# UnaryPlus/raytrace

Measured on AMD Instinct MI355X. Metric: Msamples/s (pixels×spp/s) + achieved HBM GB/s, Cornell-box 600×600, higher is better.
Workload: dtype f64; 1 GPU; cornell 600x600 200spp depth 50; width=600, height=600, spp=200, max_depth=50, parallelism=rows interleaved over 1 GPU(s), row_block 1

## Files before the change

### raytrace_amd/csrc/rt_build.cpp

```cpp
#include <algorithm>
#include <cmath>
#include <cstdarg>
#include <cstdio>
#include <cstdlib>
#include <cstring>
#include <optional>
#include <utility>

#include "../../include/rt.h"
#include "rt_bvh.h"
#include "rt_encode8_table.h"
#include "rt_internal.h"
#include "rt_kernel_class.h"

const char* rt_knob(const char* name) {
  const char* on = std::getenv("RT_AMD_EXPERIMENTS");
  if (!on || !*on || std::atoi(on) == 0) return nullptr;
  return std::getenv(name);
}

namespace {

struct d3 {
  double x, y, z;
// ... 1020 lines not shown
  P.tile_rows = rows;
  return RT_OK;
}

template <class R>
int rt_host_match_target(const HostScene& H, int variant, KernelParamsT<R>& P) {
  P.target_defer = 0;
  P.target_rec = -1;
  if (!H.flat || (variant & RT_VAR_BASE) != RT_VAR_FLAT || (variant & (RT_VAR_MATS | RT_VAR_MEDIA))) return 0;
  if (const char* e = rt_knob("RT_AMD_TARGET_DEFER"))
    if (atoi(e) == 0) return 0;
  if (rt_knob("RT_AMD_VARIANT")) return 0;
  const HostArraysT<R>& A = H.arrays<R>();
  if (P.n_targets != 1 || H.n_media != 0 || A.flat_recs.empty() || A.prim_shade.empty()) return 0;
  const DevFlatSet& S = H.flat_sets[0];
  const DevTargetT<R>& T = P.targets[0];
  for (int k = S.first; k < S.end_quad; ++k) {
    const R* f = A.flat_recs.data() + 16 * (size_t)k;
    if (std::memcmp(f, T.n, 3 * sizeof(R)) || std::memcmp(f + 4, T.q, 3 * sizeof(R)) ||
        std::memcmp(f + 8, T.wa, 3 * sizeof(R)) || std::memcmp(f + 12, T.wb, 3 * sizeof(R)))
      continue;
    int kf, slot;
    std::memcpy(&kf, f + 3, 4);
    std::memcpy(&slot, f + 11, 4);
    if (kf != 1 || slot < 0 || slot >= (int)A.prim_shade.size()) continue;
    if (A.prim_shade[slot].kind >= 2) continue;
    P.target_defer = 1;
    P.target_rec = k;
    return 1;
  }
  return 0;
}

template <class R>
SceneRecordsT<R> rt_host_records(const HostScene& H) {
  const HostArraysT<R>& A = H.arrays<R>();
  SceneRecordsT<R> r;
  r.nodes = H.nodes.data(), r.perlin_perm = H.perlin_perm.data();
  r.prims = A.prims.data(), r.prim_uv = A.prim_uv.data(), r.motions = A.motions.data();
  r.uvframes = A.uvframes.data(), r.texels = A.texels.data(), r.perlin_grad = A.perlin_grad.data();
  r.flat_recs = A.flat_recs.data(), r.prim_shade = A.prim_shade.data(), r.mats = A.mats.data();
  r.texs = A.texs.data(), r.boxes = A.boxes.data(), r.instances = A.instances.data();
  return r;
}

template <class R>
int rt_host_render_params(const HostScene& H, int variant, const SceneRecordsT<R>& r, const rt_camera_settings* cs,
                          uint64_t seed, const rt_exec* ex, const LaunchInputs& L, KernelParamsT<R>& P,
                          std::string& err) {
  constexpr bool f64 = sizeof(R) == 8;
  const bool flat = (variant & RT_VAR_BASE) == RT_VAR_FLAT;
  std::memset(&P, 0, sizeof P);
  if (int rc = rt_host_make_params(cs, seed, ex, P, err)) return rc;
  P.nodes = r.nodes, P.perlin_perm = r.perlin_perm;
  P.prims = r.prims, P.prim_uv = r.prim_uv, P.motions = r.motions, P.uvframes = r.uvframes, P.texels = r.texels;
  P.perlin_grad = r.perlin_grad, P.flat_recs = r.flat_recs, P.prim_shade = r.prim_shade, P.mats = r.mats;
  P.texs = r.texs, P.boxes = r.boxes, P.instances = r.instances;
  P.surface_root = H.surface_root;
  P.leaf_exit_pct = f64 ? H.leaf_exit_pct64 : H.leaf_exit_pct;
  P.surface_prefix = !flat && H.n_nodes > 0 ? 1 : 0;
  P.n_media = H.n_media;
  for (int k = 0; k < H.n_media; ++k) P.media[k] = H.arrays<R>().media[k];
  for (int k = 0; k <= RT_MAX_MEDIA; ++k) P.flat_sets[k] = H.flat_sets[k];
  P.stack_depth = rt_host_stack_depth(H);
  P.lds_nodes = L.lds_nodes;
  P.n_prims = H.n_prims;
  P.pool_shift = L.pool_shift ? L.pool_shift : L.lone && flat ? 6 : 0;
  rt_host_plan_work(P, L.resident_lanes, flat, L.lone);
  if (L.flat_ring) rt_host_plan_ring(P, variant, L.lone, L.pool_shift, L.resident_lanes);
  P.trav_exit_pct = f64 ? H.trav_exit_pct64 : H.trav_exit_pct;
  P.out_frame_rows = L.out_frame_rows;
  P.sample0 = L.sample0;
  rt_host_match_target(H, variant, P);
  return RT_OK;
}
#define RT_INSTANTIATE(R)                                                                                           \
  template int rt_host_match_target<R>(const HostScene&, int, KernelParamsT<R>&);                                   \
  template SceneRecordsT<R> rt_host_records<R>(const HostScene&);                                                   \
  template int rt_host_render_params<R>(const HostScene&, int, const SceneRecordsT<R>&, const rt_camera_settings*, \
                                        uint64_t, const rt_exec*, const LaunchInputs&, KernelParamsT<R>&, std::string&);
RT_INSTANTIATE(float)
RT_INSTANTIATE(double)
#undef RT_INSTANTIATE

bool rt_host_media_late(const HostScene& H) {
  if (H.n_media == 0) return false;
  for (int m = 0; m < H.n_media; ++m) {
    const DevMediumT<double>& M = H.f64.media[m];
    if (!M.alias_surface && !(M.root < 0 && M.root != RT_EMPTY_ROOT)) return false;
  }
  return true;
}

FastDiv rt_host_fastdiv(uint32_t d) {
  FastDiv f{0u, 0, d, 0};
  if (d <= 1) return f;
  int l = 0;
  while ((1ull << l) < d) ++l;
  f.m = (uint32_t)((((1ull << 32) * ((1ull << l) - d)) / d) + 1);
  f.s = l - 1;
  return f;
}

template <class R>
void rt_host_plan_work(KernelParamsT<R>& P, long long resident_lanes, bool two_sizes, bool lone) {
  P.div_width = rt_host_fastdiv((uint32_t)P.cam.width);
  P.div_block = rt_host_fastdiv((uint32_t)P.row_block);
  const bool pool_given = P.pool_shift >= 4;
  if (!pool_given) P.pool_shift = __builtin_ctz(RT_POOL);
// ... 109 lines not shown
```

### raytrace_amd/csrc/rt_internal.h

```cpp
#pragma once
#include <stdint.h>

#include <string>
#include <vector>

#ifndef RT_BLOCK
#define RT_BLOCK 64
#endif
#ifndef RT_BLOCK_BVH
#define RT_BLOCK_BVH 256
#endif
#define RT_MAX_NODES (1 << 26)
#define RT_STACK_DEPTH 64
#define RT_MAX_MEDIA 8
#define RT_MAX_TARGETS 8
#ifndef RT_LEAF_MAX
#define RT_LEAF_MAX 8
#endif
#ifndef RT_POOL
#define RT_POOL 128
#endif
#ifndef RT_AGG_SLOTS_FLAT
#define RT_AGG_SLOTS_FLAT 8
#endif
#ifndef RT_AGG_PIX_FLAT
#define RT_AGG_PIX_FLAT 17
#endif
#ifndef RT_AGG_SLOTS_FLAT_F64
#define RT_AGG_SLOTS_FLAT_F64 7
#endif
#ifndef RT_AGG_PIX_FLAT_F64
#define RT_AGG_PIX_FLAT_F64 22
#endif
#ifndef RT_AGG_SLOTS_BVH
#define RT_AGG_SLOTS_BVH 4
#endif
#ifndef RT_AGG_PIX_BVH
#define RT_AGG_PIX_BVH 5
#endif
#define RT_RING_LANES 64
#define RT_RING_AGG_PIX 8
#define RT_RING_AGG_SLOTS_F64 6
#define RT_RING_AGG_SLOTS_F32 5
#ifndef RT_BIG_CHUNK_MAX
#define RT_BIG_CHUNK_MAX 16
#endif
#ifndef RT_BIG_CHUNK_MAX_ASYNC
#define RT_BIG_CHUNK_MAX_ASYNC 64
#endif
#ifndef RT_TAIL_ITEMS_F64
#define RT_TAIL_ITEMS_F64 16
#endif
#ifndef RT_TAIL_ITEMS_F32
#define RT_TAIL_ITEMS_F32 32
#endif
#ifndef RT_TAIL_ITEMS_ASYNC
#define RT_TAIL_ITEMS_ASYNC 8
#endif
#define RT_LEAF_SHIFT 6
#define RT_FLAT_MAX 32
#define RT_LDS_PRIMS_MAX 256
#define RT_PREFIX_MAX 16
#ifndef RT_PREFIX_AREA
#define RT_PREFIX_AREA 0.1
#endif
#ifndef RT_PREFIX_SHRINK
#define RT_PREFIX_SHRINK 0.25
#endif
#define RT_EMPTY_ROOT ((int)0x80000000)
#ifndef RT_GRID_RESERVE
#define RT_GRID_RESERVE 0
#endif
#define RT_INST_FLAG 0x40000000
#define RT_INST_EXIT 0x7FFFFFFF

#define RT_VAR_FLAT 0
// ... 136 lines not shown
  int chunk;
  int n_chunks;
  int n_items;
  int big_chunk;
  int n_big_chunks;
  int big_items;
  int small_start;
  FastDiv div_big, div_small;
  int agg_big, agg_small;
  int pool_shift;
  int stack_depth;
  int lds_nodes;
  int trav_exit_pct;
  int leaf_exit_pct;
  int n_prims;
  int surface_root;
  int surface_prefix;
  int n_media;
  int n_targets;
  R rem_prob;
  DevMediumT<R> media[RT_MAX_MEDIA];
  DevFlatSet flat_sets[1 + RT_MAX_MEDIA];
  DevTargetT<R> targets[RT_MAX_TARGETS];
  DevCameraT<R> cam;
  uint32_t key0, key1;
  int n_shards, shard, row_block, tile_rows;
  int out_frame_rows;
  FastDiv div_width, div_block;
  int sample0;
  int target_defer;
  int target_rec;
  int cam_defocus;
  int flat_ring;
};
using DevMaterial = DevMaterialT<float>;
using DevTexture = DevTextureT<float>;
using DevMedium = DevMediumT<float>;
using DevBox = DevBoxT<float>;
using DevTarget = DevTargetT<float>;
using DevCamera = DevCameraT<float>;
using DevInstance = DevInstanceT<float>;
using KernelParams = KernelParamsT<float>;
using KernelParams64 = KernelParamsT<double>;

#define RT_FIX_SCALE 4294967296.0
#define RT_ACC_WORDS(R) (sizeof(R) == 8 ? 6 : 3)

template <class R>
struct HostArraysT {
  std::vector<R> prims, prim_uv, motions, uvframes, texels, perlin_grad;
  std::vector<R> flat_recs;
  std::vector<DevMaterialT<R>> prim_shade, mats;
  std::vector<DevTextureT<R>> texs;
  std::vector<DevBoxT<R>> boxes;
  std::vector<DevInstanceT<R>> instances;
  DevMediumT<R> media[RT_MAX_MEDIA];
};
struct HostScene {
  std::vector<float> nodes;
  std::vector<int> perlin_perm;
  std::vector<int> prim_mat;
  HostArraysT<float> f32;
  HostArraysT<double> f64;
  int surface_root = RT_EMPTY_ROOT;
  int n_media = 0;
  DevFlatSet flat_sets[1 + RT_MAX_MEDIA] = {};
// ... 30 lines not shown
                    int stack_depth);
inline int rt_host_stack_depth(const HostScene& H) { return H.max_depth > 1 ? H.max_depth : 1; }
template <class R>
int rt_host_make_params(const rt_camera_settings* cs, uint64_t seed, const rt_exec* ex, KernelParamsT<R>& P,
                        std::string& err);
template <class R>
struct SceneRecordsT {
  const float* nodes = nullptr;
  const int* perlin_perm = nullptr;
  const R *prims = nullptr, *prim_uv = nullptr, *motions = nullptr, *uvframes = nullptr, *texels = nullptr;
  const R *perlin_grad = nullptr, *flat_recs = nullptr;
  const DevMaterialT<R>*prim_shade = nullptr, *mats = nullptr;
  const DevTextureT<R>* texs = nullptr;
  const DevBoxT<R>* boxes = nullptr;
  const DevInstanceT<R>* instances = nullptr;
};
template <class R>
SceneRecordsT<R> rt_host_records(const HostScene& H);
struct LaunchInputs {
  long long resident_lanes = 0;
  int lds_nodes = 0;
  bool lone = false;
  int sample0 = 0, out_frame_rows = 0;
  int pool_shift = 0;
  bool flat_ring = false;
};
template <class R>
int rt_host_render_params(const HostScene& H, int variant, const SceneRecordsT<R>& records,
                          const rt_camera_settings* cs, uint64_t seed, const rt_exec* ex, const LaunchInputs& L,
                          KernelParamsT<R>& P, std::string& err);
template <class R>
int rt_host_match_target(const HostScene& H, int variant, KernelParamsT<R>& P);
template <class R>
void rt_host_plan_work(KernelParamsT<R>& P, long long resident_lanes, bool two_sizes, bool lone = false);
template <class R>
bool rt_host_plan_ring(KernelParamsT<R>& P, int variant, bool lone, int pool_shift = 0, long long resident_lanes = 0);
FastDiv rt_host_fastdiv(uint32_t d);
void rt_host_encode8_thresholds(int encoding, double* thr);

int rt_render_resident_blocks(const KernelParams*, int device, int stack_depth, int variant, int lds_nodes);
int rt_render_resident_blocks(const KernelParams64*, int device, int stack_depth, int variant, int lds_nodes);
int rt_launch_render(const KernelParams& p, int grid_blocks, int variant, void* stream);
int rt_launch_render(const KernelParams64& p, int grid_blocks, int variant, void* stream);
int rt_launch_resolve(const KernelParams& p, void* stream);
int rt_launch_resolve(const KernelParams64& p, void* stream);
int rt_launch_features(const KernelParams& p, int variant, unsigned long long* feat, int n_feat, void* stream);
int rt_launch_features(const KernelParams64& p, int variant, unsigned long long* feat, int n_feat, void* stream);
struct rt_ray;
struct rt_hit;
int rt_launch_query(const KernelParams& p, int variant, const rt_ray* rays, rt_hit* hits, const int* prim_mat, long long n,
                    int flags, void* stream);
int rt_launch_query(const KernelParams64& p, int variant, const rt_ray* rays, rt_hit* hits, const int* prim_mat,
                    long long n, int flags, void* stream);
struct rt_adaptive_rec;
int rt_launch_list(const KernelParams& p, int variant, const rt_adaptive_rec* list, const int* n_list, int n_samples,
                   int chunk, void* stream);
int rt_launch_list(const KernelParams64& p, int variant, const rt_adaptive_rec* list, const int* n_list, int n_samples,
                   int chunk, void* stream);
#if defined(RT_PHASE_PROF)
int rt_prof_read_kernel(const KernelParams*, unsigned long long* out, int n);
int rt_prof_read_kernel(const KernelParams64*, unsigned long long* out, int n);
#endif
#if defined(RT_WAVE_STAMPS)
int rt_stamps_read_kernel(const KernelParams*, unsigned long long* out, int n_waves);
int rt_stamps_read_kernel(const KernelParams64*, unsigned long long* out, int n_waves);
#endif
// ... 3 lines not shown
```

### raytrace_amd/csrc/rt_kernel_class.h

```cpp
#pragma once
#include <stddef.h>
#include <type_traits>
#include "rt_internal.h"

struct KernelClass {
  int var, tex, media; bool mats, inst; int leaf; bool narrow;
};

#ifndef RT_WAVES_FLAT
#define RT_WAVES_FLAT 7
#endif
#ifndef RT_WAVES_FLAT_NOISE
#define RT_WAVES_FLAT_NOISE 5
#endif
#ifndef RT_WAVES_BVH
#define RT_WAVES_BVH 5
#endif
#ifndef RT_WAVES_FLAT_TEX0
#define RT_WAVES_FLAT_TEX0 8
#endif
#ifndef RT_WAVES_BVH_LITE
#define RT_WAVES_BVH_LITE 6
#endif
#ifndef RT_WAVES64_FLAT_LITE
// ... 65 lines not shown
#endif
constexpr bool rt_class_acc_lds(bool f64, KernelClass c) {
  return RT_ACC_IN_LDS && c.var != RT_VAR_FLAT && (f64 || !c.media);
}

constexpr bool rt_class_agg_wide(bool f64, KernelClass c) { return f64 || c.media == 0; }
constexpr int rt_class_agg_slots(bool f64, KernelClass c) {
  return c.var != RT_VAR_FLAT ? RT_AGG_SLOTS_BVH : rt_class_agg_wide(f64, c) ? RT_AGG_SLOTS_FLAT_F64 : RT_AGG_SLOTS_FLAT;
}
constexpr int rt_class_agg_pix(bool f64, KernelClass c) {
  return c.var != RT_VAR_FLAT ? RT_AGG_PIX_BVH : rt_class_agg_wide(f64, c) ? RT_AGG_PIX_FLAT_F64 : RT_AGG_PIX_FLAT;
}
static_assert(RT_AGG_SLOTS_FLAT < 255 && RT_AGG_SLOTS_FLAT_F64 < 255 && RT_AGG_SLOTS_BVH < 255,
              "slot + 1 must fit the 8 bits of rt_trace.h ItemCtx::tp");
constexpr int rt_acc_words(bool f64) { return f64 ? RT_ACC_WORDS(double) : RT_ACC_WORDS(float); }
constexpr int rt_class_agg_bytes(bool f64, KernelClass c) {
  return rt_class_agg_slots(f64, c) * (rt_class_agg_pix(f64, c) * rt_acc_words(f64) * 8 + 2 * 4);
}
constexpr size_t rt_class_fixed_lds(bool f64, KernelClass c) {
  const size_t block = (size_t)rt_class_block(f64, c);
  return (rt_class_acc_lds(f64, c) ? rt_acc_words(f64) * 8 * block : 0) + rt_class_agg_bytes(f64, c) * (block / 64);
}
constexpr size_t rt_class_lds_bytes(bool f64, KernelClass c, int stack_depth, int lds_nodes) {
  return rt_class_fixed_lds(f64, c) +
         (c.var == RT_VAR_FLAT ? 0 : (size_t)(stack_depth + 1) * rt_class_block(f64, c) * sizeof(int) + (size_t)lds_nodes * 64);
}

constexpr KernelClass rt_ring_class() { return KernelClass{RT_VAR_FLAT, 0, 0, false, false, 0, false}; }
constexpr bool rt_class_has_ring(KernelClass c) {
  return c.var == RT_VAR_FLAT && c.tex == 0 && c.media == 0 && !c.mats && !c.inst;
}
constexpr int rt_ring_agg_slots(bool f64) { return f64 ? RT_RING_AGG_SLOTS_F64 : RT_RING_AGG_SLOTS_F32; }
constexpr int rt_ring_agg_bytes(bool f64) { return rt_ring_agg_slots(f64) * (RT_RING_AGG_PIX * rt_acc_words(f64) * 8 + 2 * 4); }
constexpr int rt_ring_ray_bytes(bool f64) { return RT_RING_LANES * (6 * (f64 ? 8 : 4) + 4 * 4); }
constexpr size_t rt_ring_lds_bytes(bool f64) { return (size_t)rt_ring_ray_bytes(f64) + rt_ring_agg_bytes(f64); }
static_assert(RT_BLOCK == RT_RING_LANES, "the ring belongs to a one-wave workgroup");
static_assert(rt_ring_lds_bytes(false) <= rt_class_fixed_lds(false, rt_ring_class()) &&
                  rt_ring_lds_bytes(true) <= rt_class_fixed_lds(true, rt_ring_class()),
              "the ring form's LDS must not exceed the legacy kernel's (same workgroups per CU)");

#ifndef RT_NOLICM_FLAT_LITE
#define RT_NOLICM_FLAT_LITE 0
#endif
#ifndef RT_NOLICM_BVH_LITE
#define RT_NOLICM_BVH_LITE 0
#endif
constexpr bool rt_class_nolicm(bool f64, KernelClass c) {
  const bool heavy = c.tex != 0 || c.media != 0 || c.mats;
  return c.var == RT_VAR_FLAT ? f64 && (RT_NOLICM_FLAT_LITE || heavy) : RT_NOLICM_BVH_LITE || heavy || c.inst;
}

#ifndef RT_LEAF_MEDIA
#define RT_LEAF_MEDIA 1
#endif
constexpr bool rt_media_late_compiled(int var) { return var == RT_VAR_BVH; }
constexpr bool rt_leaf_compiled(int var, int tex, int media, bool inst, int leaf) {
  if (leaf == 0) return true;
  if (var != RT_VAR_BVH || inst) return false;
  return media ? RT_LEAF_MEDIA && tex == 0 && leaf == 1 : true;
}
constexpr bool rt_class_compiled(bool f64, KernelClass c) {
  if (c.var == RT_VAR_BVH_LOCKSTEP && !RT_LOCKSTEP_KERNELS) return false;
  if (c.var != RT_VAR_BVH && c.inst) return false;
  if (c.media == 2 && !rt_media_late_compiled(c.var)) return false;
  return rt_leaf_compiled(c.var, c.tex, c.media, c.inst, c.leaf) && (!c.narrow || rt_class_has_twin(f64, c));
}

// ... 40 lines not shown
```

### raytrace_amd/csrc/rt_render_kernel.h

```cpp
#include <hip/hip_runtime.h>
#include <stdint.h>

#include <type_traits>

#include "rt_kernel_class.h"
#include "rt_trace.h"

namespace RT_NS {

#if defined(RT_WAVE_STAMPS)
#define RT_STAMP_WAVES 16384
static __device__ unsigned long long rt_stamp_buf[4 * RT_STAMP_WAVES];
#endif

namespace {

static_assert(RT_POOL >= 64, "a refill must cover every lane of a wave");
#ifndef RT_QUEUES
#define RT_QUEUES 4
#endif
#ifndef RT_QUEUE_INTERLEAVE
#define RT_QUEUE_INTERLEAVE 1
#endif
static_assert((RT_QUEUES & (RT_QUEUES - 1)) == 0 && RT_QUEUES <= 8, "RT_QUEUES: a power of two, at most 8 (workspace)");
// ... 272 lines not shown
    rt_stamp_buf[4 * wave + 1] = work.t_drain;                                                    \
    rt_stamp_buf[4 * wave + 2] = wall_clock64();                                                  \
    rt_stamp_buf[4 * wave + 3] = (unsigned long long)__builtin_amdgcn_s_getreg((4 << 0) | (31 << 11)) << 32 | \
                                 (unsigned)__builtin_amdgcn_s_getreg((20 << 0) | (3 << 11));      \
  }
#else
#define RT_STAMP_END(work)
#endif
  if constexpr (kVar == RT_VAR_FLAT) {
    WaveWork<kSlots, kPix, true> work(P, wave, waves, agg);
    overflow = lane_loop_lockstep<true, kTex, kMedia != 0, kMats>(P, work, Trav{nullptr, 0, nullptr}, P.prims, acc);
    work.finish();
    RT_STAMP_END(work)
  } else {
    v4f* lds_nodes = reinterpret_cast<v4f*>(smem_rest + (P.stack_depth + 1) * block_nodes);
    const float4* src = reinterpret_cast<const float4*>(P.nodes);
    for (int i = threadIdx.x; i < 4 * P.lds_nodes; i += block_copy) {
      const float4 q = src[i];
      lds_nodes[i] = v4f{q.x, q.y, q.z, q.w};
    }
    __syncthreads();
    WaveWork<kSlots, kPix, RT_KARGS_WORK_BVH> work(P, wave, waves, agg);
    const Trav W{smem_rest + threadIdx.x, block_stack, lds_nodes};
    if constexpr (kVar == RT_VAR_BVH_LOCKSTEP)
      overflow = lane_loop_lockstep<false, kTex, kMedia != 0, kMats>(P, work, W, P.prims, acc);
    else
      overflow = lane_loop_bvh<kTex, kMedia, kMats, kInst, kLeaf>(P, work, W, P.prims, acc);
    work.finish();
    RT_STAMP_END(work)
  }
  if (overflow) atomicOr(P.status, 1);
}

#if !RT_TU_NOLICM
__global__ __launch_bounds__(RT_BLOCK) __attribute__((amdgpu_waves_per_eu(rt_class_waves(RT_F64, rt_ring_class()))))
void rt_render_kernel_ring(KernelParams P) {
  extern __shared__ int smem[];
  real* ring_od = reinterpret_cast<real*>(smem);
  uint32_t* ring_meta = reinterpret_cast<uint32_t*>(ring_od + 6 * RT_RING_LANES);
  unsigned long long* agg = reinterpret_cast<unsigned long long*>(ring_meta + 4 * RT_RING_LANES);
  constexpr int kAggBytes = rt_ring_agg_bytes(RT_F64);
  for (int i = (int)__lane_id(); i < kAggBytes / 8; i += 64) agg[i] = 0ull;
  WaveWork<rt_ring_agg_slots(RT_F64), RT_RING_AGG_PIX, true> work(P, (int)blockIdx.x, (int)gridDim.x, agg);
  lane_loop_flat_ring(P, work, ring_od, ring_meta);
  work.finish();
}
#endif

#ifndef RT_KERNEL_ONLY
#if !RT_TU_NOLICM
__global__ __launch_bounds__(256) void rt_resolve_kernel(const long long* __restrict__ accum,
                                                         const unsigned int* __restrict__ nanflag,
                                                         real* __restrict__ out, int n_pixels, int spp, double scale,
                                                         int width, int frame_rows, int n_shards, int shard,
                                                         int row_block) {
  const int i = blockIdx.x * 256 + threadIdx.x;
  if (i >= n_pixels) return;
  size_t w = 3 * (size_t)i + blockIdx.y;
  if (frame_rows > 0) {
    const int t = i / width, px = i - t * width;
    const int g = ((t / row_block) * n_shards + shard) * row_block + t % row_block;
    if (g >= frame_rows) return;
    w = 3 * ((size_t)g * width + px) + blockIdx.y;
  }
  const bool bad = nanflag[i] != 0u;
#if RT_F64
  (void)scale;
  const long long* a = accum + 6 * (size_t)i + blockIdx.y;
  const double sum = ((double)a[0] + (double)(unsigned long long)a[3] * (1.0 / RT_FIX_SCALE)) * (1.0 / RT_FIX_SCALE);
  out[w] = bad ? __builtin_nan("") : sum / (double)spp;
#else
  (void)spp;
  out[w] = bad ? __builtin_nanf("") : (float)((double)accum[3 * (size_t)i + blockIdx.y] * scale);
// ... 10 lines not shown
    return nullptr;
  });
}
render_fn render_kernel_nolicm(int variant);
template <class T, size_t N>
static int diag_read(T (&buf)[N], unsigned long long* out, size_t n) {
  if (hipMemcpyFromSymbol(out, HIP_SYMBOL(buf), n * sizeof(T)) != hipSuccess) return -1;
  void* p = nullptr;
  if (hipGetSymbolAddress(&p, HIP_SYMBOL(buf)) != hipSuccess) return -1;
  return hipMemset(p, 0, sizeof(buf)) == hipSuccess ? 0 : -1;
}
int diag_read_nolicm(int which, unsigned long long* out, size_t n);
static int diag_read_this_tu(int which, unsigned long long* out, size_t n) {
  (void)which, (void)out, (void)n;
#if defined(RT_PHASE_PROF)
  if (which == 0) return diag_read(rt_prof_buf, out, n);
#endif
#if defined(RT_WAVE_STAMPS)
  if (which == 1) return diag_read(rt_stamp_buf, out, n);
#endif
  return -1;
}
#if RT_TU_NOLICM
int diag_read_nolicm(int which, unsigned long long* out, size_t n) { return diag_read_this_tu(which, out, n); }
#endif
static int diag_read_both(int which, unsigned long long* out, size_t n) {
  if (hipDeviceSynchronize() != hipSuccess || diag_read_this_tu(which, out, n)) return -1;
  unsigned long long* other = new unsigned long long[n];
  const int rc = diag_read_nolicm(which, other, n);
  for (size_t k = 0; k < n && rc == 0; ++k) out[k] += other[k];
  delete[] other;
  return rc;
}
#if RT_TU_NOLICM
render_fn render_kernel_nolicm(int variant) { return render_kernel_this_tu(variant); }
#else
static render_fn render_kernel_of(int variant) {
  const render_fn f = render_kernel_this_tu(variant);
  return f ? f : render_kernel_nolicm(variant);
}
#endif

#endif
}
#if !defined(RT_KERNEL_ONLY) && !RT_TU_NOLICM

int rt_render_resident_blocks(const KernelParamsT<RT_NS::real>*, int device, int stack_depth, int variant,
                              int lds_nodes) {
  using namespace RT_NS;
  int per_cu = 0, cus = 0;
  const KernelClass c = rt_class_of(RT_F64, variant);
  size_t lds = rt_class_lds_bytes(RT_F64, c, stack_depth, lds_nodes);
  if (lds > 65536 && hipFuncSetAttribute((const void*)render_kernel_of(variant),
                                         hipFuncAttributeMaxDynamicSharedMemorySize, (int)lds) != hipSuccess)
    return -1;
  hipError_t e =
      hipOccupancyMaxActiveBlocksPerMultiprocessor(&per_cu, render_kernel_of(variant), rt_class_block(RT_F64, c), lds);
  if (e != hipSuccess) return -1;
  if (hipDeviceGetAttribute(&cus, hipDeviceAttributeMultiprocessorCount, device) != hipSuccess) return -1;
  if (per_cu < 1) per_cu = 1;
  return per_cu * cus;
}

int rt_launch_render(const KernelParamsT<RT_NS::real>& p, int grid_blocks, int variant, void* stream) {
  using namespace RT_NS;
  if (p.n_items <= 0 || grid_blocks <= 0) return 0;
  const KernelClass c = rt_class_of(RT_F64, variant);
  const int block = rt_class_block(RT_F64, c);
  long long need = ((long long)p.n_items + block - 1) / block;
  int grid = need < grid_blocks ? (int)need : grid_blocks;
  if (p.flat_ring) {
    if (!rt_class_has_ring(c)) return -1;
    hipLaunchKernelGGL(rt_render_kernel_ring, dim3(grid), dim3(block), rt_ring_lds_bytes(RT_F64), (hipStream_t)stream, p);
    return hipGetLastError() == hipSuccess ? 0 : -1;
  }
  size_t lds = rt_class_lds_bytes(RT_F64, c, p.stack_depth, p.lds_nodes);
  hipLaunchKernelGGL(render_kernel_of(variant), dim3(grid), dim3(block), lds, (hipStream_t)stream, p);
  return hipGetLastError() == hipSuccess ? 0 : -1;
}

#if defined(RT_PHASE_PROF)
int rt_prof_read_kernel(const KernelParamsT<RT_NS::real>*, unsigned long long* out, int n) {
  using namespace RT_NS;
  if (n > PF_N) n = PF_N;
  return diag_read_both(0, out, (size_t)n) == 0 ? n : -1;
}
#endif

#if defined(RT_WAVE_STAMPS)
int rt_stamps_read_kernel(const KernelParamsT<RT_NS::real>*, unsigned long long* out, int n_waves) {
  using namespace RT_NS;
  if (n_waves > RT_STAMP_WAVES) n_waves = RT_STAMP_WAVES;
  return diag_read_both(1, out, 4 * (size_t)n_waves) == 0 ? n_waves : -1;
}
#endif

int rt_launch_resolve(const KernelParamsT<RT_NS::real>& p, void* stream) {
  using namespace RT_NS;
  int n = p.tile_rows * p.cam.width;
  if (n <= 0) return 0;
  hipLaunchKernelGGL(rt_resolve_kernel, dim3((n + 255) / 256, 3), dim3(256), 0, (hipStream_t)stream,
                     (const long long*)p.accum, p.nanflag, p.out, n, p.cam.spp, 1.0 / (RT_FIX_SCALE * (double)p.cam.spp),
                     p.cam.width, p.out_frame_rows, p.n_shards, p.shard, p.row_block);
  return hipGetLastError() == hipSuccess ? 0 : -1;
}
#endif
// ... 1 lines not shown
```

### raytrace_amd/csrc/rt_trace.h

```cpp
#ifndef RT_TRACE_COMMON_H
#define RT_TRACE_COMMON_H
#include <stdint.h>

#include "../../include/rt.h"
#include "rt_internal.h"
#include "rt_sincos_table.h"

#ifdef RT_HOST_EMU
#include <cmath>
#include <cstring>
#define RT_FN static inline
#define RT_FN_SPEC inline
namespace rt_emu {
inline int f2i(float f) {
  int i;
  std::memcpy(&i, &f, 4);
  return i;
}
extern thread_local long long counters[4];
}
#define RT_F2I(f) rt_emu::f2i(f)
#define RT_COUNT(i) (++rt_emu::counters[i])
#define RT_ANY(x) (x)
#define RT_BALLOT_COUNT(x) ((x) ? 1 : 0)
// ... 1101 lines not shown
template <bool kDefer>
RT_FN void closest_flat(const KernelParams& P, int set, const RayCtx& R, real tmin, Closest& C, real* apdf = nullptr) {
  {
    const DevFlatSet& S = P.flat_sets[set];
    const real tmin_up = float_up(tmin);
    for (int b = S.box_first; b < S.box_end; ++b) test_box<true>((const RT_CAS DevBox*)P.boxes + b, R, tmin_up, C);
    int k = S.first;
    const RT_CAS PrimRec64* rp = (const RT_CAS PrimRec64*)P.flat_recs + k;
    for (; k < S.end_quad; ++k, ++rp) {
      if constexpr (kDefer) {
        if (k == P.target_rec) {
          real term;
          test_static<RT_PRIM_CLASS_QUAD>(ld_rec64(rp), R, tmin, tmin_up, C, 0, &term);
          *apdf = RFMA(P.targets[0].prob_icr, term, *apdf);
          continue;
        }
      }
      test_static<RT_PRIM_CLASS_QUAD>(ld_rec64(rp), R, tmin, tmin_up, C);
    }
    for (; k < S.end_tri; ++k, ++rp) test_static<RT_PRIM_CLASS_TRI>(ld_rec64(rp), R, tmin, tmin_up, C);
    for (; k < S.end_sphere; ++k, ++rp) test_static<RT_PRIM_CLASS_SPHERE>(ld_rec64(rp), R, tmin, tmin_up, C);
    for (; k < S.end; ++k, ++rp) test_rec<true>(P, ld_rec64(rp), k, R, tmin, tmin_up, C);
#if RT_F64
    if (C.t < kInf) C.prim = C.ord;
#else
    const uint32_t hi = (uint32_t)(C.key >> 32);
    if (hi < 0x7f800000u) {
      C.t = __builtin_bit_cast(real, hi);
      C.prim = (int)(uint32_t)C.key;
    }
#endif
  }
}
template <>
RT_FN_SPEC void closest<true>(const KernelParams& P, cfp prims, int root, int set, const RayCtx& R, real tmin, Closest& C,
                         const Trav& W, int* overflow) {
  (void)prims;
  (void)root;
  (void)W;
  (void)overflow;
  closest_flat<false>(P, set, R, tmin, C);
}

template <>
RT_FN_SPEC void closest<false>(const KernelParams& P, cfp prims, int root, int set, const RayCtx& R, real tmin,
                          Closest& C, const Trav& W, int* overflow) {
  TravState S;
  trav_begin(S, root, tmin);
  if (set == 0) prefix_hits(P, prims, R, tmin, S.C);
  while (!trav_done(S)) trav_round(P, R, S, W, *overflow RT_PROF_NULLARG);
  C = S.C;
}

#ifndef RT_KARGS_OPAQUE
#define RT_KARGS_OPAQUE 1
#endif
#if defined(RT_HOST_EMU) || !RT_KARGS_OPAQUE
#define RT_KARGS(P0) (P0)
#else
RT_FN const KernelParams& rt_kargs() {
  const RT_CAS KernelParams* pp = (const RT_CAS KernelParams*)__builtin_amdgcn_kernarg_segment_ptr();
  asm volatile("" : "+s"(pp));
  return *(const KernelParams*)pp;
}
#define RT_KARGS(P0) rt_kargs()
#endif
// ... 85 lines not shown
    medium_event(P, m, pix, sample, seg, lo, hi, tbest, hit_medium);
  }
}

RT_FN f3 normalize_fused(f3 v) {
#ifdef RT_HOST_EMU
  return normalize(v);
#else
  const real l = RFMA(v.z, v.z, RFMA(v.y, v.y, v.x * v.x));
#if RT_F64
  if (RABS(l) <= RL(1e-12) || RABS(RL(1.0) - l) <= RL(1e-12)) return v;
#else
  if (l <= RL(1e-12)) return v;
#endif
  return RT_RSQRT(l) * v;
#endif
}
template <bool kFlatLoop = false>
RT_FN f3 normal_plus_unit_vector(f3 n, uint32_t a, uint32_t b, f3& uu) {
  real z = RL(1.0) - RL(2.0) * u01(a);
  real r = RT_SQRT(RMAX(RL(0.0), RL(1.0) - z * z));
  real s, c;
  if constexpr (kFlatLoop)
    RT_SINCOS_TURNS_S(u01(b), &s, &c);
  else
    RT_SINCOS_TURNS(u01(b), &s, &c);
  uu = mk3(r * c, r * s, z);
#ifdef RT_HOST_EMU
  return n + uu;
#else
  return mk3(RFMA(r, c, n.x), RFMA(r, s, n.y), n.z + z);
#endif
}
template <bool kMats, bool kEarly, class... Defer>
RT_FN bool mixture_scatter(const KernelParams& P, const HitInfo& h, const RayCtx& R, const u4& w, const DevMaterial& Mt,
                           bool hemi, f3 tex, f3& newdir, f3& Tf, Defer... apdf) {
  constexpr bool kDefer = sizeof...(Defer) == 1;
  real cr = u01(w.x);
  int choice = -1;
  for (int k = 0; k < P.n_targets; ++k) {
    if (cr < P.targets[k].thresh) {
      choice = k;
      break;
    }
  }
  f3 dir;
  if constexpr (kDefer) {
    if (choice < 0) {
      f3 uu;
      dir = normal_plus_unit_vector<true>(h.n, w.y, w.z, uu);
    } else {
      const DevTarget& Tg = P.targets[choice];
      f3 lp = ld3(Tg.q) + u01(w.y) * ld3(Tg.u) + u01(w.z) * ld3(Tg.v);
      dir = lp - h.p;
    }
    dir = normalize_fused(dir);
  } else if (choice < 0) {
    f3 uu;
    const f3 nu = normal_plus_unit_vector(h.n, w.y, w.z, uu);
    dir = hemi ? normalize_fused(nu) : uu;
  } else {
    const DevTarget& Tg = P.targets[choice];
    f3 lp = ld3(Tg.q) + u01(w.y) * ld3(Tg.u) + u01(w.z) * ld3(Tg.v);
    dir = normalize_fused(lp - h.p);
  }
  real pdf1 = hemi ? dot(dir, h.n) * (RL(1.0) / kPi) : RL(0.25) / kPi;
  if constexpr (kEarly)
    if (hemi && pdf1 <= RL(0.0)) return false;
  if constexpr (kDefer && !kMats && !kEarly) {
    if (P.target_defer) {
      *(apdf, ...) = P.rem_prob * pdf1;
      Tf = pdf1 * tex;
      newdir = dir;
      return !(hemi && pdf1 <= RL(0.0));
    }
  }
  real mix = RL(0.0);
  for (int k = 0; k < P.n_targets; ++k) {
    real tt, rinv;
    if (target_hit(P.targets[k], h.p, dir, tt, rinv)) mix += P.targets[k].prob_icr * (tt * tt * RABS(rinv));
  }
  real pdf = P.rem_prob * pdf1 + mix;
  f3 f = tex;
  if constexpr (kMats) {
    if (Mt.kind == 3) {
      real mu0 = -dot(R.d, h.n), mu1 = dot(dir, h.n);
      f = (RL(0.25) * RT_RCP(mu0 + mu1)) * f;
    } else if (Mt.kind == 9) {
      real g = Mt.param, mu = dot(R.d, dir);
      real base = RL(1.0) + g * g - RL(2.0) * g * mu;
      f = ((RL(1.0) - g * g) * RT_RCP(base * RT_SQRT(base))) * f;
    }
  }
  Tf = (pdf1 * RT_RCP(pdf)) * f;
  newdir = dir;
  return !(hemi && pdf1 <= RL(0.0));
}

RT_FN f3 background(const KernelParams& P, f3 d) {
  f3 bg = ld3(P.cam.bg0);
  if (P.cam.bg_kind == 1) {
    real a = RL(0.5) * (d.y + RL(1.0));
    bg = (RL(1.0) - a) * bg + a * ld3(P.cam.bg1);
  }
  return bg;
}
template <bool kInst>
RT_FN const RT_CAS DevMaterial* hit_material(const KernelParams& P, int best, int best_inst, int hit_medium) {
  const RT_CAS DevMaterial* Mp = hit_medium >= 0
                                     ? (const RT_CAS DevMaterial*)P.mats + P.media[hit_medium].material
                                     : (const RT_CAS DevMaterial*)P.prim_shade + best;
  if constexpr (kInst) {
    if (hit_medium < 0 && best_inst >= 0) {
      const int im = inst_rec(P, best_inst)->material;
      if (im >= 0) Mp = (const RT_CAS DevMaterial*)P.mats + im;
    }
  }
  return Mp;
}
template <bool kInst>
RT_FN HitInfo surface_info_world(const KernelParams& P, cfp prims, int best, int best_inst, const RayCtx& R, real t,
                                 bool need_uv) {
  if constexpr (kInst) {
    if (best_inst >= 0) {
      const RT_CAS DevInstance* I = inst_rec(P, best_inst);
      RayCtx Ro = R;
      Ro.o = inst_to_object(I, R.o, true);
// ... 328 lines not shown
        closest<kFlat>(P, prims, M.root, m + 1, R, t1, C2, TW, &overflow);
        if (C2.prim < 0) continue;
        lo = t1;
        hi = C2.t;
      } else {
        lo = kTmin;
        hi = t1;
      }
      medium_event(P, m, I.pix, I.sample, seg, lo, hi, tbest, hit_medium);
    }
    RT_PROF_MARK(PF_TRAV);
    f3 L = mk3(RL(0.), RL(0.), RL(0.));
    bool ended;
    if constexpr (kDefer)
      ended = shade<kTex, kMats, false>(P, prims, I.pix, I.sample, seg, tbest, best, hit_medium, R, L, T, -1, &apdf);
    else
      ended = shade<kTex, kMats>(P, prims, I.pix, I.sample, seg, tbest, best, hit_medium, R, L, T);
    if (ended) {
#ifdef RT_HOST_EMU
      apdf = RT_NAN;
#endif
      RT_HOOK_SAMPLE(I.pix, I.sample, L);
      acc_sample(acc, L, bad);
      alive = false;
      ++I.sample;
    }
    RT_PROF_MARK(PF_SHADE);
  }
  RT_PROF_FLUSH
  return overflow;
}

#ifndef RT_HOST_EMU
RT_FN int wave_prefix(unsigned long long m) {
  return (int)__builtin_amdgcn_mbcnt_hi((uint32_t)(m >> 32), __builtin_amdgcn_mbcnt_lo((uint32_t)m, 0u));
}
template <class Work>
RT_FN void commit_sample_ring(Work& work, int tpk, f3 L) {
  Acc a;
  acc_clear(a);
  bool bad = false;
  acc_sample(a, L, bad);
  work.commit_ring(tpk, a, bad);
}
template <class Work>
RT_FN void flush_ring(Work& work, const real* ring_od, const uint32_t* ring_meta, int filled) {
  constexpr int kN = RT_RING_LANES;
  __builtin_amdgcn_wave_barrier();
  const int i = (int)__lane_id();
  if (i < filled) {
    const int tag = (int)ring_meta[3 * kN + i];
    if (tag != -1) commit_sample_ring(work, tag, mk3(ring_od[i], ring_od[kN + i], ring_od[2 * kN + i]));
  }
  __builtin_amdgcn_wave_barrier();
}
template <class Work>
RT_FN void lane_loop_flat_ring(const KernelParams& P0, Work& work, real* ring_od, uint32_t* ring_meta) {
  constexpr int kN = RT_RING_LANES;
  int cnt = 0;
  int filled = 0;
  bool drained = false;
  bool alive = false;
  uint32_t pix = 0u;
  int sample = 0, tpk = -1, seg = 0;
  f3 T = mk3(RL(1.), RL(1.), RL(1.));
  real apdf = RL(1.);
  RayCtx R;
  ray_clear(R);
  RT_PROF_DECL
  for (;;) {
    const KernelParams& P = RT_KARGS(P0);
    const bool need = !alive;
    const unsigned long long m = __ballot(need);
    RT_PROF_ADD(PF_ITERS, 1);
    RT_PROF_ADD(PF_CAM_LANES, (int)__popcll(m));
    if (m != 0ull) {
      const int rank = wave_prefix(m);
      int want = (int)__popcll(m), base = 0;
      for (;;) {
        const int take = want < cnt ? want : cnt;
        const int k = rank - base;
        if (need && k >= 0 && k < take) {
          const int e = cnt - 1 - k;
          R.o = mk3(ring_od[e], ring_od[kN + e], ring_od[2 * kN + e]);
          R.d = mk3(ring_od[3 * kN + e], ring_od[4 * kN + e], ring_od[5 * kN + e]);
          R.time_w = ring_meta[e];
          pix = ring_meta[kN + e];
          sample = (int)ring_meta[2 * kN + e];
          const int held = tpk;
          tpk = (int)ring_meta[3 * kN + e];
          ring_od[e] = T.x, ring_od[kN + e] = T.y, ring_od[2 * kN + e] = T.z;
          ring_meta[3 * kN + e] = (uint32_t)held;
          R.self_gid = -1;
          T = mk3(RL(1.), RL(1.), RL(1.));
          seg = 0;
          alive = true;
        }
        cnt -= take;
        base += take;
        want -= take;
        if (want == 0 || drained) break;
        RT_PROF_ADD(PF_FRONT_LANES, kN);
        flush_ring(work, ring_od, ring_meta, filled);
        int aslot;
        const int got = work.grab(true, aslot);
        const bool in = got < P.n_items;
        ItemCtx J{-1, 0, 0, 0u, 0u};
        const bool ok = in && open_item<true>(P, got, J);
        const int jt = work.tag_ring(J.tp, aslot);
        work.skip_ring(in && !ok, jt);
        const unsigned long long vm = __ballot(ok);
        if (ok) {
          RayCtx C;
          camera_ray_flat(P, J.pix, J.sample, J.pxgy, C);
          const int e = wave_prefix(vm);
          ring_od[e] = C.o.x, ring_od[kN + e] = C.o.y, ring_od[2 * kN + e] = C.o.z;
          ring_od[3 * kN + e] = C.d.x, ring_od[4 * kN + e] = C.d.y, ring_od[5 * kN + e] = C.d.z;
          ring_meta[e] = C.time_w;
          ring_meta[kN + e] = J.pix;
          ring_meta[2 * kN + e] = (uint32_t)J.sample;
          ring_meta[3 * kN + e] = (uint32_t)jt;
        }
        __builtin_amdgcn_wave_barrier();
        filled = cnt = (int)__popcll(vm);
        drained = __ballot(in) != ~0ull;
      }
    }
    RT_PROF_MARK(PF_FRONT);
    if (!alive) break;
    Closest C = no_hit();
    closest_flat<true>(P, 0, R, kTmin, C, &apdf);
    if (P.target_defer) T = (seg == 0 ? RL(1.) : RT_RCP(apdf)) * T;
    RT_PROF_MARK(PF_TRAV);
    f3 L = mk3(RL(0.), RL(0.), RL(0.));
    if (shade<0, false, false>(P, cf(P.prims), pix, sample, seg, C.t, C.prim, -1, R, L, T, -1, &apdf)) {
      T = L;
      alive = false;
    }
    RT_PROF_MARK(PF_SHADE);
  }
  if (tpk != -1) commit_sample_ring(work, tpk, T);
  flush_ring(work, ring_od, ring_meta, filled);
  RT_PROF_FLUSH
// ... 198 lines not shown
```

Baseline: 18240 Msamples/s.

## Shade primary hits in ring refill with screen-space culling of boxes and quads

The ring refill now traces and shades the camera ray's first bounce when the batch is generated. It stores the scatter weight and the hit primitive in extra LDS ring slots, so the main loop resumes at segment 1. Primary intersection tests skip boxes and quads whose host-computed screen-space bounding rectangle does not contain the pixel, using a wave-uniform any-lane check. This adds LDS per ring and moves the f64 ring kernel into the no-LICM translation unit. It risks register pressure and correctness issues in the deferred-weight handling.

```diff
diff --git a/raytrace_amd/csrc/rt_build.cpp b/raytrace_amd/csrc/rt_build.cpp
--- a/raytrace_amd/csrc/rt_build.cpp
+++ b/raytrace_amd/csrc/rt_build.cpp
@@ -1076,6 +1076,76 @@
   return 0;
 }
 
+namespace {
+constexpr uint32_t kCullAllLo = 0u, kCullAllHi = 0xffffffffu;
+bool solve3(const d3* m, d3 b, d3& x) {
+  const double det = dot(m[0], cross(m[1], m[2]));
+  if (!(std::fabs(det) > 0) || !std::isfinite(det)) return false;
+  const d3 c0 = cross(m[1], m[2]), c1 = cross(m[2], m[0]), c2 = cross(m[0], m[1]);
+  x = divs(smul(b.x, c0) + smul(b.y, c1) + smul(b.z, c2), det);
+  return std::isfinite(x.x) && std::isfinite(x.y) && std::isfinite(x.z);
+}
+template <class R>
+void cull_rect(const KernelParamsT<R>& P, const d3* corners, int n, uint32_t* out) {
+  out[0] = kCullAllLo, out[1] = kCullAllHi;
+  const d3 center = {(double)P.cam.center[0], (double)P.cam.center[1], (double)P.cam.center[2]};
+  const d3 pu = {(double)P.cam.pixel_u[0], (double)P.cam.pixel_u[1], (double)P.cam.pixel_u[2]};
+  const d3 pv = {(double)P.cam.pixel_v[0], (double)P.cam.pixel_v[1], (double)P.cam.pixel_v[2]};
+  const d3 w0 = d3{(double)P.cam.top_left[0], (double)P.cam.top_left[1], (double)P.cam.top_left[2]} - center;
+  const d3 rows[3] = {{pu.x, pv.x, w0.x}, {pu.y, pv.y, w0.y}, {pu.z, pv.z, w0.z}};
+  double a0 = INFINITY, a1 = -INFINITY, b0 = INFINITY, b1 = -INFINITY;
+  for (int i = 0; i < n; ++i) {
+    d3 s;
+    if (!solve3(rows, corners[i] - center, s)) return;
+    if (!(s.z > 1e-9)) return;
+    const double a = s.x / s.z, b = s.y / s.z;
+    if (!std::isfinite(a) || !std::isfinite(b)) return;
+    a0 = std::min(a0, a), a1 = std::max(a1, a), b0 = std::min(b0, b), b1 = std::max(b1, b);
+  }
+  const double x0 = std::floor(a0) - 1, x1 = std::floor(a1) + 1, y0 = std::floor(b0) - 1, y1 = std::floor(b1) + 1;
+  if (x1 < 0 || y1 < 0 || x0 > 65535 || y0 > 65535) {
+    out[0] = 1u, out[1] = 0u;
+    return;
+  }
+  const uint32_t px0 = (uint32_t)std::max(0.0, x0), px1 = (uint32_t)std::min(65535.0, x1);
+  const uint32_t gy0 = (uint32_t)std::max(0.0, y0), gy1 = (uint32_t)std::min(65535.0, y1);
+  out[0] = gy0 << 16 | px0;
+  out[1] = gy1 << 16 | px1;
+}
+}
+template <class R>
+void rt_host_cull_rects(const HostScene& H, KernelParamsT<R>& P) {
+  for (int j = 0; j < RT_CULL_BOXES; ++j) P.cull_box[j][0] = kCullAllLo, P.cull_box[j][1] = kCullAllHi;
+  for (int j = 0; j < RT_CULL_QUADS; ++j) P.cull_quad[j][0] = kCullAllLo, P.cull_quad[j][1] = kCullAllHi;
+  if (!H.flat || P.cam_defocus) return;
+  if (const char* e = rt_knob("RT_AMD_PRIMARY_CULL"))
+    if (atoi(e) == 0) return;
+  const HostArraysT<R>& A = H.arrays<R>();
+  const DevFlatSet& S = H.flat_sets[0];
+  for (int b = S.box_first; b < S.box_end && b - S.box_first < RT_CULL_BOXES && b < (int)A.boxes.size(); ++b) {
+    const DevBoxT<R>& B = A.boxes[b];
+    const d3 rows[3] = {{(double)B.a0[0], (double)B.a0[1], (double)B.a0[2]},
+                        {(double)B.a1[0], (double)B.a1[1], (double)B.a1[2]},
+                        {(double)B.a2[0], (double)B.a2[1], (double)B.a2[2]}};
+    d3 c[8];
+    bool ok = true;
+    for (int i = 0; i < 8 && ok; ++i)
+      ok = solve3(rows, d3{(double)B.sc[0] + (i & 1), (double)B.sc[1] + (i >> 1 & 1), (double)B.sc[2] + (i >> 2 & 1)}, c[i]);
+    if (ok) cull_rect(P, c, 8, P.cull_box[b - S.box_first]);
+  }
+  for (int k = S.first; k < S.end_quad && k - S.first < RT_CULL_QUADS && 16 * (size_t)(k + 1) <= A.flat_recs.size(); ++k) {
+    const R* f = A.flat_recs.data() + 16 * (size_t)k;
+    const d3 rows[3] = {{(double)f[8], (double)f[9], (double)f[10]},
+                        {(double)f[12], (double)f[13], (double)f[14]},
+                        {(double)f[0], (double)f[1], (double)f[2]}};
+    const d3 q = {(double)f[4], (double)f[5], (double)f[6]};
+    d3 u, v;
+    if (!solve3(rows, d3{1, 0, 0}, u) || !solve3(rows, d3{0, 1, 0}, v)) continue;
+    const d3 c[4] = {q, q + u, q + v, q + u + v};
+    cull_rect(P, c, 4, P.cull_quad[k - S.first]);
+  }
+}
+
 template <class R>
 SceneRecordsT<R> rt_host_records(const HostScene& H) {
   const HostArraysT<R>& A = H.arrays<R>();
@@ -1116,9 +1186,11 @@
   P.out_frame_rows = L.out_frame_rows;
   P.sample0 = L.sample0;
   rt_host_match_target(H, variant, P);
+  rt_host_cull_rects(H, P);
   return RT_OK;
 }
 #define RT_INSTANTIATE(R)                                                                                           \
+  template void rt_host_cull_rects<R>(const HostScene&, KernelParamsT<R>&);                                         \
   template int rt_host_match_target<R>(const HostScene&, int, KernelParamsT<R>&);                                   \
   template SceneRecordsT<R> rt_host_records<R>(const HostScene&);                                                   \
   template int rt_host_render_params<R>(const HostScene&, int, const SceneRecordsT<R>&, const rt_camera_settings*, \
diff --git a/raytrace_amd/csrc/rt_internal.h b/raytrace_amd/csrc/rt_internal.h
--- a/raytrace_amd/csrc/rt_internal.h
+++ b/raytrace_amd/csrc/rt_internal.h
@@ -42,6 +42,12 @@
 #define RT_RING_AGG_PIX 8
 #define RT_RING_AGG_SLOTS_F64 6
 #define RT_RING_AGG_SLOTS_F32 5
+#ifndef RT_RING_PRIMARY_F64
+#define RT_RING_PRIMARY_F64 1
+#endif
+#define RT_RING_PRIMARY_F32 0
+#define RT_CULL_BOXES 8
+#define RT_CULL_QUADS 8
 #ifndef RT_BIG_CHUNK_MAX
 #define RT_BIG_CHUNK_MAX 16
 #endif
@@ -244,6 +250,8 @@
   int target_rec;
   int cam_defocus;
   int flat_ring;
+  uint32_t cull_box[RT_CULL_BOXES][2];
+  uint32_t cull_quad[RT_CULL_QUADS][2];
 };
 using DevMaterial = DevMaterialT<float>;
 using DevTexture = DevTextureT<float>;
@@ -340,6 +348,8 @@
 template <class R>
 int rt_host_match_target(const HostScene& H, int variant, KernelParamsT<R>& P);
 template <class R>
+void rt_host_cull_rects(const HostScene& H, KernelParamsT<R>& P);
+template <class R>
 void rt_host_plan_work(KernelParamsT<R>& P, long long resident_lanes, bool two_sizes, bool lone = false);
 template <class R>
 bool rt_host_plan_ring(KernelParamsT<R>& P, int variant, bool lone, int pool_shift = 0, long long resident_lanes = 0);
diff --git a/raytrace_amd/csrc/rt_kernel_class.h b/raytrace_amd/csrc/rt_kernel_class.h
--- a/raytrace_amd/csrc/rt_kernel_class.h
+++ b/raytrace_amd/csrc/rt_kernel_class.h
@@ -121,7 +121,10 @@
 }
 constexpr int rt_ring_agg_slots(bool f64) { return f64 ? RT_RING_AGG_SLOTS_F64 : RT_RING_AGG_SLOTS_F32; }
 constexpr int rt_ring_agg_bytes(bool f64) { return rt_ring_agg_slots(f64) * (RT_RING_AGG_PIX * rt_acc_words(f64) * 8 + 2 * 4); }
-constexpr int rt_ring_ray_bytes(bool f64) { return RT_RING_LANES * (6 * (f64 ? 8 : 4) + 4 * 4); }
+constexpr bool rt_ring_primary(bool f64) { return f64 ? RT_RING_PRIMARY_F64 != 0 : RT_RING_PRIMARY_F32 != 0; }
+constexpr int rt_ring_reals(bool f64) { return rt_ring_primary(f64) ? 7 : 6; }
+constexpr int rt_ring_words(bool f64) { return rt_ring_primary(f64) ? 5 : 4; }
+constexpr int rt_ring_ray_bytes(bool f64) { return RT_RING_LANES * (rt_ring_reals(f64) * (f64 ? 8 : 4) + rt_ring_words(f64) * 4); }
 constexpr size_t rt_ring_lds_bytes(bool f64) { return (size_t)rt_ring_ray_bytes(f64) + rt_ring_agg_bytes(f64); }
 static_assert(RT_BLOCK == RT_RING_LANES, "the ring belongs to a one-wave workgroup");
 static_assert(rt_ring_lds_bytes(false) <= rt_class_fixed_lds(false, rt_ring_class()) &&
diff --git a/raytrace_amd/csrc/rt_render_kernel.h b/raytrace_amd/csrc/rt_render_kernel.h
--- a/raytrace_amd/csrc/rt_render_kernel.h
+++ b/raytrace_amd/csrc/rt_render_kernel.h
@@ -328,13 +328,14 @@
   if (overflow) atomicOr(P.status, 1);
 }
 
-#if !RT_TU_NOLICM
+#define RT_RING_NOLICM (RT_F64 ? RT_RING_PRIMARY_F64 : RT_RING_PRIMARY_F32)
+#if RT_TU_NOLICM == RT_RING_NOLICM
 __global__ __launch_bounds__(RT_BLOCK) __attribute__((amdgpu_waves_per_eu(rt_class_waves(RT_F64, rt_ring_class()))))
 void rt_render_kernel_ring(KernelParams P) {
   extern __shared__ int smem[];
   real* ring_od = reinterpret_cast<real*>(smem);
-  uint32_t* ring_meta = reinterpret_cast<uint32_t*>(ring_od + 6 * RT_RING_LANES);
-  unsigned long long* agg = reinterpret_cast<unsigned long long*>(ring_meta + 4 * RT_RING_LANES);
+  uint32_t* ring_meta = reinterpret_cast<uint32_t*>(ring_od + rt_ring_reals(RT_F64) * RT_RING_LANES);
+  unsigned long long* agg = reinterpret_cast<unsigned long long*>(ring_meta + rt_ring_words(RT_F64) * RT_RING_LANES);
   constexpr int kAggBytes = rt_ring_agg_bytes(RT_F64);
   for (int i = (int)__lane_id(); i < kAggBytes / 8; i += 64) agg[i] = 0ull;
   WaveWork<rt_ring_agg_slots(RT_F64), RT_RING_AGG_PIX, true> work(P, (int)blockIdx.x, (int)gridDim.x, agg);
@@ -411,6 +412,16 @@
   delete[] other;
   return rc;
 }
+#if RT_RING_NOLICM
+render_fn ring_kernel_nolicm();
+#if RT_TU_NOLICM
+render_fn ring_kernel_nolicm() { return rt_render_kernel_ring; }
+#else
+static render_fn ring_kernel_of() { return ring_kernel_nolicm(); }
+#endif
+#elif !RT_TU_NOLICM
+static render_fn ring_kernel_of() { return rt_render_kernel_ring; }
+#endif
 #if RT_TU_NOLICM
 render_fn render_kernel_nolicm(int variant) { return render_kernel_this_tu(variant); }
 #else
@@ -450,7 +461,7 @@
   int grid = need < grid_blocks ? (int)need : grid_blocks;
   if (p.flat_ring) {
     if (!rt_class_has_ring(c)) return -1;
-    hipLaunchKernelGGL(rt_render_kernel_ring, dim3(grid), dim3(block), rt_ring_lds_bytes(RT_F64), (hipStream_t)stream, p);
+    hipLaunchKernelGGL(ring_kernel_of(), dim3(grid), dim3(block), rt_ring_lds_bytes(RT_F64), (hipStream_t)stream, p);
     return hipGetLastError() == hipSuccess ? 0 : -1;
   }
   size_t lds = rt_class_lds_bytes(RT_F64, c, p.stack_depth, p.lds_nodes);
diff --git a/raytrace_amd/csrc/rt_trace.h b/raytrace_amd/csrc/rt_trace.h
--- a/raytrace_amd/csrc/rt_trace.h
+++ b/raytrace_amd/csrc/rt_trace.h
@@ -1157,6 +1157,38 @@
 #endif
   }
 }
+RT_FN bool cull_inside(const uint32_t (&r)[2], int px, int gy) {
+  return px >= (int)(r[0] & 0xffffu) && px <= (int)(r[1] & 0xffffu) && gy >= (int)(r[0] >> 16) && gy <= (int)(r[1] >> 16);
+}
+RT_FN void closest_flat_primary(const KernelParams& P, const RayCtx& R, uint32_t pxgy, Closest& C) {
+  const DevFlatSet& S = P.flat_sets[0];
+  const real tmin = kTmin, tmin_up = float_up(tmin);
+  const int gy = (int)(pxgy >> 16), px = (int)(pxgy & 0xffffu);
+  for (int b = S.box_first; b < S.box_end; ++b) {
+    const int j = b - S.box_first;
+    if (j < RT_CULL_BOXES && !RT_ANY(cull_inside(P.cull_box[j], px, gy))) continue;
+    test_box<true>((const RT_CAS DevBox*)P.boxes + b, R, tmin_up, C);
+  }
+  int k = S.first;
+  const RT_CAS PrimRec64* rp = (const RT_CAS PrimRec64*)P.flat_recs + k;
+  for (; k < S.end_quad; ++k, ++rp) {
+    const int j = k - S.first;
+    if (j < RT_CULL_QUADS && !RT_ANY(cull_inside(P.cull_quad[j], px, gy))) continue;
+    test_static<RT_PRIM_CLASS_QUAD>(ld_rec64(rp), R, tmin, tmin_up, C);
+  }
+  for (; k < S.end_tri; ++k, ++rp) test_static<RT_PRIM_CLASS_TRI>(ld_rec64(rp), R, tmin, tmin_up, C);
+  for (; k < S.end_sphere; ++k, ++rp) test_static<RT_PRIM_CLASS_SPHERE>(ld_rec64(rp), R, tmin, tmin_up, C);
+  for (; k < S.end; ++k, ++rp) test_rec<true>(P, ld_rec64(rp), k, R, tmin, tmin_up, C);
+#if RT_F64
+  if (C.t < kInf) C.prim = C.ord;
+#else
+  const uint32_t hi = (uint32_t)(C.key >> 32);
+  if (hi < 0x7f800000u) {
+    C.t = __builtin_bit_cast(real, hi);
+    C.prim = (int)(uint32_t)C.key;
+  }
+#endif
+}
 template <>
 RT_FN_SPEC void closest<true>(const KernelParams& P, cfp prims, int root, int set, const RayCtx& R, real tmin, Closest& C,
                          const Trav& W, int* overflow) {
@@ -1308,6 +1340,13 @@
   return mk3(RFMA(r, c, n.x), RFMA(r, s, n.y), n.z + z);
 #endif
 }
+struct DeferW {
+  real w;
+};
+RT_FN void defer_put(real* a, real apdf, real) { *a = apdf; }
+RT_FN void defer_put(DeferW* a, real, real w) { a->w = w; }
+RT_FN void defer_put_w(real*, real) {}
+RT_FN void defer_put_w(DeferW* a, real w) { a->w = w; }
 template <bool kMats, bool kEarly, class... Defer>
 RT_FN bool mixture_scatter(const KernelParams& P, const HitInfo& h, const RayCtx& R, const u4& w, const DevMaterial& Mt,
                            bool hemi, f3 tex, f3& newdir, f3& Tf, Defer... apdf) {
@@ -1345,7 +1384,7 @@
     if (hemi && pdf1 <= RL(0.0)) return false;
   if constexpr (kDefer && !kMats && !kEarly) {
     if (P.target_defer) {
-      *(apdf, ...) = P.rem_prob * pdf1;
+      defer_put(apdf..., P.rem_prob * pdf1, pdf1);
       Tf = pdf1 * tex;
       newdir = dir;
       return !(hemi && pdf1 <= RL(0.0));
@@ -1368,7 +1407,9 @@
       f = ((RL(1.0) - g * g) * RT_RCP(base * RT_SQRT(base))) * f;
     }
   }
-  Tf = (pdf1 * RT_RCP(pdf)) * f;
+  const real wq = pdf1 * RT_RCP(pdf);
+  if constexpr (kDefer) defer_put_w(apdf..., wq);
+  Tf = wq * f;
   newdir = dir;
   return !(hemi && pdf1 <= RL(0.0));
 }
@@ -1763,6 +1804,10 @@
 }
 
 #ifndef RT_HOST_EMU
+#ifndef RT_RING_PRIMARY
+#define RT_RING_PRIMARY (RT_F64 ? RT_RING_PRIMARY_F64 : RT_RING_PRIMARY_F32)
+#endif
+static_assert(RT_LDS_PRIMS_MAX < 0xffff, "a ring entry packs the leaf left and the hit primitive in 16 bits each");
 RT_FN int wave_prefix(unsigned long long m) {
   return (int)__builtin_amdgcn_mbcnt_hi((uint32_t)(m >> 32), __builtin_amdgcn_mbcnt_lo((uint32_t)m, 0u));
 }
@@ -1788,6 +1833,7 @@
 template <class Work>
 RT_FN void lane_loop_flat_ring(const KernelParams& P0, Work& work, real* ring_od, uint32_t* ring_meta) {
   constexpr int kN = RT_RING_LANES;
+  constexpr bool kPrimary = RT_RING_PRIMARY != 0;
   int cnt = 0;
   int filled = 0;
   bool drained = false;
@@ -1822,9 +1868,19 @@
           tpk = (int)ring_meta[3 * kN + e];
           ring_od[e] = T.x, ring_od[kN + e] = T.y, ring_od[2 * kN + e] = T.z;
           ring_meta[3 * kN + e] = (uint32_t)held;
-          R.self_gid = -1;
-          T = mk3(RL(1.), RL(1.), RL(1.));
-          seg = 0;
+          if constexpr (kPrimary) {
+            const real w = ring_od[6 * kN + e];
+            const uint32_t gp = ring_meta[4 * kN + e];
+            const RT_CAS DevMaterial* Mp = (const RT_CAS DevMaterial*)P.prim_shade + (gp & 0xffffu);
+            R.self_gid = (int)(gp >> 16) - 1;
+            T = w * f3{Mp->c0[0], Mp->c0[1], Mp->c0[2]};
+            apdf = P.rem_prob * w;
+            seg = 1;
+          } else {
+            R.self_gid = -1;
+            T = mk3(RL(1.), RL(1.), RL(1.));
+            seg = 0;
+          }
           alive = true;
         }
         cnt -= take;
@@ -1840,6 +1896,38 @@
         const bool ok = in && open_item<true>(P, got, J);
         const int jt = work.tag_ring(J.tp, aslot);
         work.skip_ring(in && !ok, jt);
+        if constexpr (kPrimary) {
+          bool go = false;
+          RayCtx C;
+          DeferW D{RL(0.)};
+          int gp = 0;
+          if (ok) {
+            camera_ray_flat(P, J.pix, J.sample, J.pxgy, C);
+            Closest H = no_hit();
+            closest_flat_primary(P, C, J.pxgy, H);
+            f3 L = mk3(RL(0.), RL(0.), RL(0.)), T1 = mk3(RL(1.), RL(1.), RL(1.));
+            int seg1 = 0;
+            go = !shade<0, false, false>(P, cf(P.prims), J.pix, J.sample, seg1, H.t, H.prim, -1, C, L, T1, -1, &D);
+            gp = (C.self_gid + 1) << 16 | H.prim;
+            if (!go) commit_sample_ring(work, jt, L);
+          }
+          const unsigned long long vm = __ballot(go);
+          if (go) {
+            const int e = wave_prefix(vm);
+            ring_od[e] = C.o.x, ring_od[kN + e] = C.o.y, ring_od[2 * kN + e] = C.o.z;
+            ring_od[3 * kN + e] = C.d.x, ring_od[4 * kN + e] = C.d.y, ring_od[5 * kN + e] = C.d.z;
+            ring_od[6 * kN + e] = D.w;
+            ring_meta[e] = C.time_w;
+            ring_meta[kN + e] = J.pix;
+            ring_meta[2 * kN + e] = (uint32_t)J.sample;
+            ring_meta[3 * kN + e] = (uint32_t)jt;
+            ring_meta[4 * kN + e] = (uint32_t)gp;
+          }
+          __builtin_amdgcn_wave_barrier();
+          filled = cnt = (int)__popcll(vm);
+          drained = __ballot(in) != ~0ull;
+          continue;
+        }
         const unsigned long long vm = __ballot(ok);
         if (ok) {
           RayCtx C;
```

After: 19390 Msamples/s (median of 6 runs). 6.3% higher.
